# eminwux/kukeon

Hardware: AMD Instinct MI355X
Metric: agent_turns_per_sec (higher is better)
Workload: dtype bf16; 1 GPU; model=llama-3-8b, global_batch=64, seq_len=3584, parallelism=dp1, sessions_per_gpu_group=64, prompt_len=512, followup_len=256, decode_len=128

## Files before the change

kukeon_amd/ops/__init__.py:

```python
from __future__ import annotations

import torch

from . import reference

_C = None
_IMPORT_ERROR: Exception | None = None


def _load() -> None:
    global _C, _IMPORT_ERROR
    try:
        from kukeon_amd import _C as ext
    except Exception as e:
        _IMPORT_ERROR = e
    else:
        _C, _IMPORT_ERROR = ext, None


_load()


def native_available() -> bool:
    if _C is None:
        _load()
    return _C is not None


def _native():
    if _C is None:
        _load()
    if _C is None:
        raise RuntimeError(
            "kukeon_amd._C (gfx950 HIP extension) is not built but an op was "
            "called on a CUDA device. Run `python -m kukeon_amd.ops.build` "
            f"(import error: {_IMPORT_ERROR})")
    return _C


def _impl(t: torch.Tensor):
    return _native() if t.is_cuda else reference


def rmsnorm(out, input, weight, eps: float) -> None:
    _impl(input).rmsnorm(out, input, weight, eps)


def fused_add_rmsnorm(input, residual, weight, eps: float) -> None:
    _impl(input).fused_add_rmsnorm(input, residual, weight, eps)


def silu_mul(out, gate_up) -> None:
    _impl(gate_up).silu_mul(out, gate_up)


def rope_kv_append(qkv, k_cache, v_cache, cos_sin, positions, slot_mapping,
                   num_q_heads: int, num_kv_heads: int, head_dim: int,
                   block_table=None) -> None:
    if block_table is None:
        block_table = torch.empty(0, dtype=torch.int32, device=qkv.device)
    _impl(qkv).rope_kv_append(qkv, k_cache, v_cache, cos_sin, positions,
                              slot_mapping, num_q_heads, num_kv_heads,
                              head_dim, block_table)


def kv_copy_blocks(k_cache, v_cache, src, dst) -> None:
    _impl(k_cache).kv_copy_blocks(k_cache, v_cache, src, dst)


def decode_advance(ids, pos, seq_lens, tokens, ring, counter) -> None:
    _impl(ids).decode_advance(ids, pos, seq_lens, tokens, ring, counter)


def paged_attention(out, q, k_cache, v_cache, block_table, seq_lens,
                    q_offset: int, num_splits: int, scale: float,
                    tmp_out, tmp_ml) -> None:
    _impl(q).paged_attention(out, q, k_cache, v_cache, block_table, seq_lens,
                             q_offset, num_splits, scale, tmp_out, tmp_ml)


DECODE_ATTN_FUSED = __import__("os").environ.get(
    "KUKEON_DECODE_ATTN_FUSED", "1") != "0"


def paged_attention_rope(out, qkv, k_cache, v_cache, cos_sin, positions,
                         block_table, seq_lens, num_q_heads: int,
                         num_kv_heads: int, num_splits: int, scale: float,
                         tmp_out, tmp_ml) -> None:
    _impl(qkv).paged_attention_rope(out, qkv, k_cache, v_cache, cos_sin,
                                    positions, block_table, seq_lens,
                                    num_q_heads, num_kv_heads, num_splits,
                                    scale, tmp_out, tmp_ml)


def check_prefix_tiles(tiles, group: int) -> None:
    reference.check_prefix_tiles(tiles, group)


def paged_attention_shared(out, q, k_cache, v_cache, block_table, seq_lens,
                           q_offset: int, num_splits: int, scale: float,
                           tmp_out, tmp_ml, prefix_blocks, tiles,
                           prefix_splits: int) -> None:
    _impl(q).paged_attention_shared(out, q, k_cache, v_cache, block_table,
                                    seq_lens, q_offset, num_splits, scale,
                                    tmp_out, tmp_ml, prefix_blocks, tiles,
                                    prefix_splits)


def paged_attention_rope_shared(out, qkv, k_cache, v_cache, cos_sin,
                                positions, block_table, seq_lens,
                                num_q_heads: int, num_kv_heads: int,
                                num_splits: int, scale: float, tmp_out,
                                tmp_ml, prefix_blocks, tiles,
                                prefix_splits: int) -> None:
    _impl(qkv).paged_attention_rope_shared(
        out, qkv, k_cache, v_cache, cos_sin, positions, block_table,
        seq_lens, num_q_heads, num_kv_heads, num_splits, scale, tmp_out,
        tmp_ml, prefix_blocks, tiles, prefix_splits)


def prefill_attention(out, q, k_cache, v_cache, block_table, seq_lens,
                      q_starts, qb_seq, qb_start, q_offset: int,
                      scale: float) -> None:
    _impl(q).prefill_attention(out, q, k_cache, v_cache, block_table,
                               seq_lens, q_starts, qb_seq, qb_start, q_offset,
                               scale)


def sample(tokens, logits, temps, top_k, top_p, seed, workspace) -> None:
    _impl(logits).sample(tokens, logits, temps, top_k, top_p, seed, workspace)


_SKINNY_WS = {}
_SKINNY_WS_RETIRED = []
_USE_SKINNY = __import__("os").environ.get("KUKEON_SKINNY_GEMM", "0")
_FUSE_SILU = __import__("os").environ.get("KUKEON_FUSE_SILU", "0") == "1"


def _skinny_wins(rows: int, N: int, K: int) -> bool:
    if _USE_SKINNY == "off":
        return False
    return N == K == 4096


def _skinny5_wins(rows: int, N: int, K: int) -> bool:
    if _USE_SKINNY == "off":
        return False
    return (N, K) in ((4096, 14336), (8192, 28672))


def _skinny_kind(x: torch.Tensor, w: torch.Tensor, fused: bool):
    rows = x.shape[0]
    if not (x.is_cuda and x.dim() == 2 and rows <= 64
            and x.dtype == torch.bfloat16):
        return None
    N, K = w.shape
    if fused:
        from kukeon_amd import parallel
        if not (parallel.tp_size() == 1 and N % 2048 == 0 and N <= 8192):
            return None
    if (N % 128 == 0 and K % 128 == 0
            and (_USE_SKINNY == "5" or _skinny5_wins(rows, N, K))):
        return "v5"
    if (N % 64 == 0 and K % 32 == 0
            and (_USE_SKINNY == "1" or _skinny_wins(rows, N, K))):
        return "v1"
    return None


_SKINNY_SPLITK = {}


def _skinny_workspace(device: torch.device, kind: str, N: int,
                      K: int) -> torch.Tensor:
    splitk = _SKINNY_SPLITK.get((kind, N, K))
    if splitk is None:
        splitk = _SKINNY_SPLITK[kind, N, K] = _native().skinny_splitk(
            kind, N, K)
    need = 64 * N * splitk
    key = (device.index or 0)
    ws = _SKINNY_WS.get(key)
    if ws is None or ws.numel() < need:
        if ws is not None:
            _SKINNY_WS_RETIRED.append(ws)
        ws = torch.empty(need, dtype=torch.float32, device=device)
        _SKINNY_WS[key] = ws
    return ws


class Fp8Weight:

    __slots__ = ("q", "scale")

    def __init__(self, q: torch.Tensor, scale: torch.Tensor):
        assert q.dtype == torch.uint8 and q.dim() == 2
        assert scale.dtype == torch.float32 and scale.shape == (q.shape[0],)
        self.q = q
        self.scale = scale

    @property
    def shape(self):
        return tuple(self.q.shape)

    @property
    def device(self) -> torch.device:
        return self.q.device

    @property
    def is_cuda(self) -> bool:
        return self.q.is_cuda

    @property
    def nbytes(self) -> int:
        return self.q.numel() + 4 * self.scale.numel()


_W8_SCRATCH = {}
_W8_SCRATCH_RETIRED = []


def _w8_scratch(device: torch.device, numel: int) -> torch.Tensor:
    key = (device.index or 0)
    buf = _W8_SCRATCH.get(key)
    if buf is None or buf.numel() < numel:
        if buf is not None:
            _W8_SCRATCH_RETIRED.append(buf)
        buf = torch.empty(numel, dtype=torch.bfloat16, device=device)
        _W8_SCRATCH[key] = buf
    return buf


def quantize_weight(w: torch.Tensor) -> Fp8Weight:
    w = w.detach().contiguous()
    N, K = w.shape
    q = torch.empty(N, K, dtype=torch.uint8, device=w.device)
    scale = torch.empty(N, dtype=torch.float32, device=w.device)
    _impl(w).quantize_fp8_rows(q, scale, w)
    if w.is_cuda:
        _w8_scratch(w.device, N * K)
    return Fp8Weight(q, scale)


def dequantize_weight(fw: Fp8Weight, out: torch.Tensor = None) -> torch.Tensor:
    if out is None:
        out = torch.empty(fw.shape, dtype=torch.bfloat16, device=fw.device)
    _impl(fw.q).dequant_fp8_rows(out, fw.q, fw.scale)
    return out


def _w8_skinny(x: torch.Tensor, fw: Fp8Weight) -> bool:
    N, K = fw.shape
    return (x.is_cuda and x.dim() == 2 and 1 <= x.shape[0] <= 64
            and x.dtype == torch.bfloat16 and x.is_contiguous()
            and N % 64 == 0 and K % 64 == 0)


def _linear_w8(x: torch.Tensor, fw: Fp8Weight) -> torch.Tensor:
    if not x.is_cuda:
        return reference.linear_w8(x, fw.q, fw.scale)
    N, K = fw.shape
    if _w8_skinny(x, fw):
        out = torch.empty(x.shape[0], N, dtype=x.dtype, device=x.device)
        ws = _skinny_workspace(x.device, "w8", N, K)
        _native().skinny_gemm_w8(out, x, fw.q, fw.scale, ws)
        return out
    w = _w8_scratch(x.device, N * K)[:N * K].view(N, K)
    _native().dequant_fp8_rows(w, fw.q, fw.scale)
    return torch.nn.functional.linear(x, w)


def linear(x: torch.Tensor, w) -> torch.Tensor:
    if isinstance(w, Fp8Weight):
        return _linear_w8(x, w)
    kind = _skinny_kind(x, w, fused=False)
    if kind is None:
        return torch.nn.functional.linear(x, w)
    N, K = w.shape
    out = torch.empty(x.shape[0], N, dtype=x.dtype, device=x.device)
    ws = _skinny_workspace(x.device, kind, N, K)
    if kind == "v5":
        _native().skinny_gemm5(out, x, w, ws)
    else:
        _native().skinny_gemm(out, x, w, ws)
    return out


def linear_add_rmsnorm(x: torch.Tensor, w: torch.Tensor,
                       residual: torch.Tensor, norm_weight: torch.Tensor,
                       eps: float) -> torch.Tensor:
    if isinstance(w, Fp8Weight):
        from kukeon_amd import parallel
        N, K = w.shape
        if (_w8_skinny(x, w) and parallel.tp_size() == 1
                and N % 2048 == 0 and N <= 8192):
            normed = torch.empty(x.shape[0], N, dtype=x.dtype,
                                 device=x.device)
            ws = _skinny_workspace(x.device, "w8", N, K)
            _native().skinny_gemm_w8_fused_norm(normed, x, w.q, w.scale, ws,
                                                residual, norm_weight, eps)
            return normed
        kind = None
    else:
        kind = _skinny_kind(x, w, fused=True)
    if kind is None:
        from kukeon_amd import parallel
        h = parallel.tp_all_reduce(linear(x, w))
        fused_add_rmsnorm(h, residual, norm_weight, eps)
        return h
    N, K = w.shape
    normed = torch.empty(x.shape[0], N, dtype=x.dtype, device=x.device)
    if kind == "v5":
        ws = _skinny_workspace(x.device, "v5_fused", N, K)
        _native().skinny_gemm5_fused_norm(normed, x, w, ws, residual,
                                          norm_weight, eps)
    else:
        ws = _skinny_workspace(x.device, "v1", N, K)
        _native().skinny_gemm_fused_norm(normed, x, w, ws, residual,
                                         norm_weight, eps)
    return normed


def mlp_down_fused(gu: torch.Tensor, w: torch.Tensor,
                   residual: torch.Tensor, norm_weight: torch.Tensor,
                   eps: float) -> torch.Tensor:
    rows = gu.shape[0]
    N, K = w.shape
    if (_FUSE_SILU and not isinstance(w, Fp8Weight) and gu.dim() == 2
            and gu.shape[1] == 2 * K
            and _skinny_kind(gu, w, fused=True) == "v5"):
        ws = _skinny_workspace(gu.device, "v5_fused", N, K)
        normed = torch.empty(rows, N, dtype=gu.dtype, device=gu.device)
        _native().skinny_gemm5_silu_fused_norm(normed, gu, w, ws,
                                               residual, norm_weight, eps)
        return normed
    act = torch.empty(rows, K, dtype=gu.dtype, device=gu.device)
    silu_mul(act, gu)
    return linear_add_rmsnorm(act, w, residual, norm_weight, eps)


def moe_router_weights(wdense, logits, k: int) -> None:
    _impl(logits).moe_router_weights(wdense, logits, k)


def moe_dense_combine(out, y, wdense) -> None:
    _impl(y).moe_dense_combine(out, y, wdense)


def moe_gather_tokens(out, input, row_map) -> None:
    _impl(input).moe_gather_tokens(out, input, row_map)


def moe_scatter_tokens(out, input, inv_map, weights, top_k: int) -> None:
    _impl(input).moe_scatter_tokens(out, input, inv_map, weights, top_k)


def moe_route_sort(topk_w, row_map, inv_map, offsets, logits, k: int) -> None:
    _impl(logits).moe_route_sort(topk_w, row_map, inv_map, offsets, logits,
                                 k)


def moe_grouped_gemm(out, a, a_rows, w, offsets) -> None:
    if a_rows is None:
        a_rows = torch.empty(0, dtype=torch.int32, device=a.device)
    _impl(a).moe_grouped_gemm(out, a, a_rows, w, offsets)
```

kukeon_amd/ops/csrc/bindings.cpp:

```cpp
#include <torch/extension.h>

namespace kukeon {
void rmsnorm(torch::Tensor out, torch::Tensor input, torch::Tensor weight,
             double eps);
void fused_add_rmsnorm(torch::Tensor input, torch::Tensor residual,
                       torch::Tensor weight, double eps);
void silu_mul(torch::Tensor out, torch::Tensor gate_up);
void rope_kv_append(torch::Tensor qkv, torch::Tensor k_cache,
                    torch::Tensor v_cache, torch::Tensor cos_sin,
                    torch::Tensor positions, torch::Tensor slot_mapping,
                    int64_t num_q_heads, int64_t num_kv_heads,
                    int64_t head_dim, torch::Tensor block_table);
void decode_advance(torch::Tensor ids, torch::Tensor pos,
                    torch::Tensor seq_lens, torch::Tensor tokens,
                    torch::Tensor ring, torch::Tensor counter);
void kv_copy_blocks(torch::Tensor k_cache, torch::Tensor v_cache,
                    torch::Tensor src, torch::Tensor dst);
void paged_attention(torch::Tensor out, torch::Tensor q, torch::Tensor k_cache,
                     torch::Tensor v_cache, torch::Tensor block_table,
                     torch::Tensor seq_lens, int64_t q_offset,
                     int64_t num_splits, double scale, torch::Tensor tmp_out,
                     torch::Tensor tmp_ml);
void paged_attention_rope(torch::Tensor out, torch::Tensor qkv,
                          torch::Tensor k_cache, torch::Tensor v_cache,
                          torch::Tensor cos_sin, torch::Tensor positions,
                          torch::Tensor block_table, torch::Tensor seq_lens,
                          int64_t num_q_heads, int64_t num_kv_heads,
                          int64_t num_splits, double scale,
                          torch::Tensor tmp_out, torch::Tensor tmp_ml);
void paged_attention_shared(torch::Tensor out, torch::Tensor q,
                            torch::Tensor k_cache, torch::Tensor v_cache,
                            torch::Tensor block_table, torch::Tensor seq_lens,
                            int64_t q_offset, int64_t num_splits, double scale,
                            torch::Tensor tmp_out, torch::Tensor tmp_ml,
                            torch::Tensor prefix_blocks, torch::Tensor tiles,
                            int64_t prefix_splits);
void paged_attention_rope_shared(
    torch::Tensor out, torch::Tensor qkv, torch::Tensor k_cache,
    torch::Tensor v_cache, torch::Tensor cos_sin, torch::Tensor positions,
    torch::Tensor block_table, torch::Tensor seq_lens, int64_t num_q_heads,
    int64_t num_kv_heads, int64_t num_splits, double scale,
    torch::Tensor tmp_out, torch::Tensor tmp_ml, torch::Tensor prefix_blocks,
    torch::Tensor tiles, int64_t prefix_splits);
void prefill_attention(torch::Tensor out, torch::Tensor q,
                       torch::Tensor k_cache, torch::Tensor v_cache,
                       torch::Tensor block_table, torch::Tensor seq_lens,
                       torch::Tensor q_starts, torch::Tensor qb_seq,
                       torch::Tensor qb_start, int64_t q_offset, double scale);
void mfma_probe(torch::Tensor out, torch::Tensor a, torch::Tensor b);
void mfma_probe16(torch::Tensor out, torch::Tensor a, torch::Tensor b);
void mfma_probe16k(torch::Tensor out, torch::Tensor a, torch::Tensor b);
void skinny_gemm2(torch::Tensor out, torch::Tensor x, torch::Tensor w,
                  torch::Tensor ws);
void skinny_gemm5(torch::Tensor out, torch::Tensor x, torch::Tensor w,
                  torch::Tensor ws);
void skinny_gemm6(torch::Tensor out, torch::Tensor x, torch::Tensor w,
                  torch::Tensor ws);
void skinny_gemm5_silu_fused_norm(torch::Tensor normed, torch::Tensor gu,
                                  torch::Tensor w, torch::Tensor ws,
                                  torch::Tensor residual, torch::Tensor nw,
                                  double eps);
void skinny_gemm(torch::Tensor out, torch::Tensor x, torch::Tensor w,
                 torch::Tensor ws);
void glds_probe(torch::Tensor out, torch::Tensor src);
int64_t skinny_splitk(const std::string& kind, int64_t N, int64_t K);
void skinny_gemm5_fused_norm(torch::Tensor normed, torch::Tensor x,
                             torch::Tensor w, torch::Tensor ws,
                             torch::Tensor residual, torch::Tensor nw,
                             double eps);
void skinny_gemm_fused_norm(torch::Tensor normed, torch::Tensor x,
                            torch::Tensor w, torch::Tensor ws,
                            torch::Tensor residual, torch::Tensor nw,
                            double eps);
void skinny_gemm_w8(torch::Tensor out, torch::Tensor x, torch::Tensor q,
                    torch::Tensor scale, torch::Tensor ws);
void skinny_gemm_w8_fused_norm(torch::Tensor normed, torch::Tensor x,
                               torch::Tensor q, torch::Tensor scale,
                               torch::Tensor ws, torch::Tensor residual,
                               torch::Tensor nw, double eps);
void quantize_fp8_rows(torch::Tensor q, torch::Tensor scale, torch::Tensor w);
void dequant_fp8_rows(torch::Tensor out, torch::Tensor q,
                      torch::Tensor scale);
void sample(torch::Tensor tokens, torch::Tensor logits, torch::Tensor temps,
            torch::Tensor top_k, torch::Tensor top_p, torch::Tensor seed,
            torch::Tensor workspace);
void moe_router_weights(torch::Tensor wdense, torch::Tensor logits,
                        long K);
void moe_dense_combine(torch::Tensor out, torch::Tensor y,
                       torch::Tensor wdense);
void moe_gather_tokens(torch::Tensor out, torch::Tensor input,
                       torch::Tensor row_map);
void moe_scatter_tokens(torch::Tensor out, torch::Tensor input,
                        torch::Tensor row_map, torch::Tensor weights,
                        int64_t top_k);
void moe_route_sort(torch::Tensor topk_w, torch::Tensor row_map,
                    torch::Tensor inv_map, torch::Tensor offsets,
                    torch::Tensor logits, long K);
void moe_grouped_gemm(torch::Tensor out, torch::Tensor a,
                      torch::Tensor a_rows, torch::Tensor w,
                      torch::Tensor offsets);
}

PYBIND11_MODULE(TORCH_EXTENSION_NAME, m) {
  m.def("rmsnorm", &kukeon::rmsnorm, "RMSNorm (bf16, gfx950)");
  m.def("fused_add_rmsnorm", &kukeon::fused_add_rmsnorm,
        "residual += input; input = rmsnorm(residual)");
  m.def("silu_mul", &kukeon::silu_mul, "out = silu(gate)*up from fused [T,2I]");
  m.def("rope_kv_append", &kukeon::rope_kv_append,
        "in-place NEOX RoPE on fused qkv + paged KV append");
  m.def("kv_copy_blocks", &kukeon::kv_copy_blocks,
        "cache[l, dst[i]] = cache[l, src[i]] for K and V, all layers, one "
        "launch");
  m.def("paged_attention", &kukeon::paged_attention,
        "decode paged attention (GQA, split-KV)");
  m.def("paged_attention_rope", &kukeon::paged_attention_rope,
        "decode paged attention with RoPE + KV append folded in");
  m.def("paged_attention_shared", &kukeon::paged_attention_shared,
        "decode paged attention, shared prefix blocks read once per tile of "
        "rows");
  m.def("paged_attention_rope_shared", &kukeon::paged_attention_rope_shared,
        "paged_attention_rope, shared prefix blocks read once per tile of "
        "rows");
  m.def("prefill_attention", &kukeon::prefill_attention,
        "varlen causal paged prefill attention (MFMA)");
  m.def("mfma_probe", &kukeon::mfma_probe,
        "32x32x16 bf16 MFMA fragment-layout probe");
  m.def("mfma_probe16", &kukeon::mfma_probe16,
        "16x16x32 bf16 MFMA fragment-layout probe");
  m.def("mfma_probe16k", &kukeon::mfma_probe16k,
        "16x16x16 (K=16) bf16 MFMA fragment-layout probe");
  m.def("skinny_gemm6", &kukeon::skinny_gemm6,
        "decode GEMM v6 (barrier-free register-x pipeline)");
  m.def("skinny_gemm5_silu_fused_norm",
        &kukeon::skinny_gemm5_silu_fused_norm,
        "silu(gate)*up + down GEMM + reduce + add + RMSNorm fused");
  m.def("skinny_gemm5", &kukeon::skinny_gemm5,
        "full-line W stream via wave-private LDS image (v5)");
  m.def("skinny_gemm2", &kukeon::skinny_gemm2,
        "G-walk hand-counted weight-streaming GEMM (v2)");
  m.def("skinny_gemm", &kukeon::skinny_gemm,
        "weight-streaming decode GEMM (M<=64)");
  m.def("skinny_splitk", &kukeon::skinny_splitk,
        "split-K factor the skinny launcher of `kind` (v1, v2, v5, v5_fused, "
        "v6, w8) uses for [N, K]; host-only",
        py::arg("kind"), py::arg("N"), py::arg("K"));
  m.def("glds_probe", &kukeon::glds_probe,
        "asm global_lds round-trip validator");
  m.def("skinny_gemm5_fused_norm", &kukeon::skinny_gemm5_fused_norm,
        "skinny5 + fused split-K reduce + residual add + RMSNorm");
  m.def("skinny_gemm_fused_norm", &kukeon::skinny_gemm_fused_norm,
        "skinny GEMM + split-K reduce + residual add + RMSNorm");
  m.def("skinny_gemm_w8", &kukeon::skinny_gemm_w8,
        "W8A16 decode GEMM: (x @ fp8(q)^T) * scale, M<=64");
  m.def("skinny_gemm_w8_fused_norm", &kukeon::skinny_gemm_w8_fused_norm,
        "W8A16 decode GEMM + split-K reduce + residual add + RMSNorm");
  m.def("quantize_fp8_rows", &kukeon::quantize_fp8_rows,
        "bf16 [N,K] -> e4m3fn bytes + per-row f32 scale (amax/448)");
  m.def("dequant_fp8_rows", &kukeon::dequant_fp8_rows,
        "out = bf16(fp8(q) * scale[n])");
  m.def("sample", &kukeon::sample, "top-k/top-p/temperature sampling");
  m.def("decode_advance", &kukeon::decode_advance,
        "on-device decode cursor advance (self-advancing graph)");
  m.def("moe_gather_tokens", &kukeon::moe_gather_tokens, "MoE permute");
  m.def("moe_router_weights", &kukeon::moe_router_weights,
        "softmax top-K renorm -> dense [T,E] weights, one launch");
  m.def("moe_dense_combine", &kukeon::moe_dense_combine,
        "out = sum_e w[t,e]*y[e,t,:], zero-weight experts skipped");
  m.def("moe_scatter_tokens", &kukeon::moe_scatter_tokens,
        "MoE unpermute + weighted combine");
  m.def("moe_route_sort", &kukeon::moe_route_sort,
        "top-k routing + stable expert sort on the device, one launch");
  m.def("moe_grouped_gemm", &kukeon::moe_grouped_gemm,
        "out[r] = a[a_rows[r]] @ w[e].T, expert row ranges from device");
}
```

kukeon_amd/ops/csrc/prefill_attn.hip:

```cpp
#include "attn_frag.h"
#include <torch/extension.h>
#include <c10/hip/HIPStream.h>

namespace kukeon {

template <int BS, bool FP8>
__global__ __launch_bounds__(256, 1) void prefill_attn_kernel(
    unsigned short* __restrict__ out,
    const unsigned short* __restrict__ q,
    const void* __restrict__ k_cache,
    const void* __restrict__ v_cache,
    const int* __restrict__ block_table,
    const int* __restrict__ seq_lens,
    const int* __restrict__ q_starts,
    const int* __restrict__ qb_seq,
    const int* __restrict__ qb_start,
    long q_stride, long q_offset, int Hq, int Hk, int max_blocks,
    int out_stride, float scale) {
  constexpr int D = 128;
  constexpr int KVT = 32;
  __shared__ __align__(16) unsigned short kbuf[KVT * D];
  __shared__ __align__(16) unsigned short vtbuf[D * KVT];

  const int s = qb_seq[blockIdx.x];
  const int qb0 = qb_start[blockIdx.x];
  const int hk = blockIdx.y;
  const int ctx = seq_lens[s];
  const int abs_start = q_starts[2 * s];
  const int row0 = q_starts[2 * s + 1] + qb0;
  const int qlen = ctx - abs_start;
  const int qn = min(32, qlen - qb0);
  if (qn <= 0) return;
  const int G = Hq / Hk;
  const int wid = threadIdx.x / WAVE;
  const int lane = threadIdx.x & (WAVE - 1);
  const int hi = lane >> 5;
  const int qcol = lane & 31;
  const int h_local = blockIdx.z * 4 + wid;
  const bool active = h_local < G;
  const int head = hk * G + (active ? h_local : 0);

  const int q_abs = abs_start + qb0 + min(qcol, qn - 1);

  unsigned int qfrag[8][4];
  {
    const long qrow = row0 + min(qcol, qn - 1);
    const unsigned short* qp = q + qrow * q_stride + q_offset + (long)head * D;
#pragma unroll
    for (int st = 0; st < 8; ++st) {
      const uint4 v = *reinterpret_cast<const uint4*>(qp + st * 16 + hi * 8);
      qfrag[st][0] = v.x; qfrag[st][1] = v.y;
      qfrag[st][2] = v.z; qfrag[st][3] = v.w;
    }
  }

  float m = -INFINITY, l_acc = 0.f;
  f32x16_t oacc[4] = {{}, {}, {}, {}};

  const int kv_limit = min(ctx, abs_start + qb0 + qn);
  const int ntiles = (kv_limit + KVT - 1) / KVT;
  const int nblocks = (ctx + BS - 1) / BS;

  for (int ti = 0; ti < ntiles; ++ti) {
    const int kvbase = ti * KVT;
    {
      __syncthreads();
      const auto* kc = reinterpret_cast<const kv_elem_t<FP8>*>(k_cache);
      const auto* vc = reinterpret_cast<const kv_elem_t<FP8>*>(v_cache);
      const int tok = threadIdx.x >> 3;
      const int d0 = (threadIdx.x & 7) * 16;
      const int kvpos = kvbase + tok;
      const int bidx = min(kvpos / BS, nblocks - 1);
      const int pblk = block_table[(long)s * max_blocks + bidx];
      const long koff = (((long)pblk * Hk + hk) * BS + (kvpos % BS)) * D;
      const int swz = (tok & 15) << 4;
#pragma unroll
      for (int c = 0; c < 2; ++c) {
        const int byte = tok * 256 + (((d0 + c * 8) * 2) ^ swz);
        *reinterpret_cast<uint4*>(reinterpret_cast<char*>(kbuf) + byte) =
            load_kv8(kc + koff + d0 + c * 8);
      }
      const int kp = threadIdx.x >> 4;
      const int vd0 = (threadIdx.x & 15) * 8;
      const int vpos0 = kvbase + 2 * kp;
      const int vpos1 = vpos0 + 1;
      const int vb0 = min(vpos0 / BS, nblocks - 1);
      const int vb1 = min(vpos1 / BS, nblocks - 1);
      const long voff0 =
          (((long)block_table[(long)s * max_blocks + vb0] * Hk + hk) * BS +
           (vpos0 % BS)) * D;
      const long voff1 =
          (((long)block_table[(long)s * max_blocks + vb1] * Hk + hk) * BS +
           (vpos1 % BS)) * D;
      uint4 r0 = load_kv8(vc + voff0 + vd0);
      uint4 r1 = load_kv8(vc + voff1 + vd0);
      if (vpos0 >= ctx) r0 = uint4{0, 0, 0, 0};
      if (vpos1 >= ctx) r1 = uint4{0, 0, 0, 0};
      const unsigned int* a0 = reinterpret_cast<const unsigned int*>(&r0);
      const unsigned int* a1 = reinterpret_cast<const unsigned int*>(&r1);
#pragma unroll
      for (int j = 0; j < 8; ++j) {
        const unsigned short e0 = (a0[j >> 1] >> ((j & 1) * 16)) & 0xffffu;
        const unsigned short e1 = (a1[j >> 1] >> ((j & 1) * 16)) & 0xffffu;
        const unsigned int packed = (unsigned)e0 | ((unsigned)e1 << 16);
        const int d = vd0 + j;
        const int byte = d * 64 + ((4 * kp) ^ ((d & 3) << 4));
        *reinterpret_cast<unsigned int*>(
            reinterpret_cast<char*>(vtbuf) + byte) = packed;
      }
      __syncthreads();
    }
    if (!active) continue;

    f32x16_t sacc = {};
#pragma unroll
    for (int st = 0; st < 8; ++st) {
      const int row = qcol;
      const int byte = row * 256 + (((st * 16 + hi * 8) * 2) ^ ((row & 15) << 4));
      const uint4 kf = *reinterpret_cast<const uint4*>(
          reinterpret_cast<const char*>(kbuf) + byte);
      sacc = __builtin_amdgcn_mfma_f32_32x32x16_bf16(
          as_frag(kf.x, kf.y, kf.z, kf.w),
          as_frag(qfrag[st][0], qfrag[st][1], qfrag[st][2], qfrag[st][3]),
          sacc, 0, 0, 0);
    }

    float sv[16];
    float tmax = -INFINITY;
#pragma unroll
    for (int r = 0; r < 16; ++r) {
      const int kvrow = (r & 3) + 8 * (r >> 2) + 4 * hi;
      const int kvpos = kvbase + kvrow;
      const bool valid = (kvpos <= q_abs) && (kvpos < ctx);
      sv[r] = valid ? sacc[r] * scale : -INFINITY;
      tmax = fmaxf(tmax, sv[r]);
    }
    tmax = fmaxf(tmax, __shfl_xor(tmax, 32, WAVE));
    const float mn = fmaxf(m, tmax);
    const float alpha = (m == -INFINITY) ? 0.f : __expf(m - mn);
    m = mn;
    float psum = 0.f;
    float p[16];
#pragma unroll
    for (int r = 0; r < 16; ++r) {
      p[r] = (sv[r] == -INFINITY) ? 0.f : __expf(sv[r] - mn);
      psum += p[r];
    }
    psum += __shfl_xor(psum, 32, WAVE);
    l_acc = l_acc * alpha + psum;
#pragma unroll
    for (int db = 0; db < 4; ++db)
#pragma unroll
      for (int r = 0; r < 16; ++r) oacc[db][r] *= alpha;

    unsigned int cp[8];
#pragma unroll
    for (int j = 0; j < 8; ++j) cp[j] = cvtpk_bf16(p[2 * j], p[2 * j + 1]);
    unsigned int pb[2][4];
#pragma unroll
    for (int c = 0; c < 2; ++c) {
      const int b0 = 4 * c;
      auto s1 = __builtin_amdgcn_permlane32_swap(cp[b0 + 0], cp[b0 + 2],
                                                 false, false);
      auto s2 = __builtin_amdgcn_permlane32_swap(cp[b0 + 1], cp[b0 + 3],
                                                 false, false);
      pb[c][0] = s1[0]; pb[c][1] = s2[0];
      pb[c][2] = s1[1]; pb[c][3] = s2[1];
    }

#pragma unroll
    for (int db = 0; db < 4; ++db) {
      const int d = db * 32 + qcol;
#pragma unroll
      for (int c = 0; c < 2; ++c) {
        const int byte = d * 64 + (((c * 32) + hi * 16) ^ ((d & 3) << 4));
        const uint4 vf = *reinterpret_cast<const uint4*>(
            reinterpret_cast<const char*>(vtbuf) + byte);
        oacc[db] = __builtin_amdgcn_mfma_f32_32x32x16_bf16(
            as_frag(vf.x, vf.y, vf.z, vf.w),
            as_frag(pb[c][0], pb[c][1], pb[c][2], pb[c][3]),
            oacc[db], 0, 0, 0);
      }
    }
  }

  if (!active || qcol >= qn) return;
  const float inv = l_acc > 0.f ? 1.f / l_acc : 0.f;
  unsigned short* orow = out + (long)(row0 + qcol) * out_stride +
                         (long)head * D;
#pragma unroll
  for (int db = 0; db < 4; ++db) {
#pragma unroll
    for (int quad = 0; quad < 4; ++quad) {
      const int d = db * 32 + quad * 8 + 4 * hi;
      const unsigned int w0 = cvtpk_bf16(oacc[db][quad * 4 + 0] * inv,
                                          oacc[db][quad * 4 + 1] * inv);
      const unsigned int w1 = cvtpk_bf16(oacc[db][quad * 4 + 2] * inv,
                                          oacc[db][quad * 4 + 3] * inv);
      *reinterpret_cast<uint2*>(orow + d) = uint2{w0, w1};
    }
  }
}

void prefill_attention(torch::Tensor out, torch::Tensor q,
                       torch::Tensor k_cache, torch::Tensor v_cache,
                       torch::Tensor block_table, torch::Tensor seq_lens,
                       torch::Tensor q_starts, torch::Tensor qb_seq,
                       torch::Tensor qb_start, int64_t q_offset, double scale) {
  const int Hk = k_cache.size(1);
  const int BS = k_cache.size(2);
  const int D = k_cache.size(3);
  const int Hq = out.size(1) / D;
  const int G = Hq / Hk;
  const int nqb = qb_seq.size(0);
  if (nqb == 0) return;
  TORCH_CHECK(D == 128, "only head_dim=128 supported");
  TORCH_CHECK(BS == 16, "kv block size must be 16");
  TORCH_CHECK(q_starts.dim() == 2 && q_starts.size(1) == 2);
  TORCH_CHECK(qb_seq.scalar_type() == torch::kInt32);
  auto stream = c10::hip::getCurrentHIPStream().stream();
  dim3 grid(nqb, Hk, (G + 3) / 4);
  const bool fp8 = k_cache.scalar_type() == torch::kUInt8;
#define PF_LAUNCH(FP8_)                                                      \
  prefill_attn_kernel<16, FP8_><<<grid, 256, 0, stream>>>(                   \
      reinterpret_cast<unsigned short*>(out.data_ptr()),                     \
      reinterpret_cast<const unsigned short*>(q.data_ptr()),                 \
      k_cache.data_ptr(), v_cache.data_ptr(), block_table.data_ptr<int>(),   \
      seq_lens.data_ptr<int>(), q_starts.data_ptr<int>(),                    \
      qb_seq.data_ptr<int>(), qb_start.data_ptr<int>(), q.stride(0),         \
      q_offset, Hq, Hk, (int)block_table.size(1), (int)out.stride(0),        \
      (float)scale)
  if (fp8) { PF_LAUNCH(true); } else { PF_LAUNCH(false); }
#undef PF_LAUNCH
  HIP_CHECK_KERNEL();
}

}
```

Before: 51.24 turns/s.

## Double-buffer KV tiles in prefill attention and remap blocks across XCDs

Adds a pipelined variant of the prefill attention kernel. It keeps two LDS buffers for the K and transposed-V tiles and prefetches the next tiles' block-table entries and raw KV into registers while the current tile's QK MFMAs run. It also raises launch_bounds occupancy to 2 blocks per CU and optionally remaps block IDs so that consecutive logical tiles land on the same XCD for better L2 locality. Both paths are on by default behind env flags. The cost is doubled shared memory and more live registers, and prefill is only one part of an agent-turn workload.

```diff
diff --git a/kukeon_amd/ops/__init__.py b/kukeon_amd/ops/__init__.py
--- a/kukeon_amd/ops/__init__.py
+++ b/kukeon_amd/ops/__init__.py
@@ -119,12 +119,25 @@
         tmp_ml, prefix_blocks, tiles, prefix_splits)
 
 
+PREFILL_ATTN_PIPELINED = __import__("os").environ.get(
+    "KUKEON_PREFILL_ATTN_PIPELINED", "1") != "0"
+PREFILL_ATTN_XCD_REMAP = __import__("os").environ.get(
+    "KUKEON_PREFILL_ATTN_XCD", "1") != "0"
+
+
 def prefill_attention(out, q, k_cache, v_cache, block_table, seq_lens,
                       q_starts, qb_seq, qb_start, q_offset: int,
                       scale: float) -> None:
-    _impl(q).prefill_attention(out, q, k_cache, v_cache, block_table,
-                               seq_lens, q_starts, qb_seq, qb_start, q_offset,
-                               scale)
+    if not q.is_cuda:
+        reference.prefill_attention(out, q, k_cache, v_cache, block_table,
+                                    seq_lens, q_starts, qb_seq, qb_start,
+                                    q_offset, scale)
+        return
+    _native().prefill_attention(out, q, k_cache, v_cache, block_table,
+                                seq_lens, q_starts, qb_seq, qb_start,
+                                q_offset, scale, PREFILL_ATTN_PIPELINED,
+                                PREFILL_ATTN_PIPELINED
+                                and PREFILL_ATTN_XCD_REMAP)
 
 
 def sample(tokens, logits, temps, top_k, top_p, seed, workspace) -> None:
diff --git a/kukeon_amd/ops/csrc/bindings.cpp b/kukeon_amd/ops/csrc/bindings.cpp
--- a/kukeon_amd/ops/csrc/bindings.cpp
+++ b/kukeon_amd/ops/csrc/bindings.cpp
@@ -46,7 +46,8 @@
                        torch::Tensor k_cache, torch::Tensor v_cache,
                        torch::Tensor block_table, torch::Tensor seq_lens,
                        torch::Tensor q_starts, torch::Tensor qb_seq,
-                       torch::Tensor qb_start, int64_t q_offset, double scale);
+                       torch::Tensor qb_start, int64_t q_offset, double scale,
+                       bool pipelined, bool xcd_remap);
 void mfma_probe(torch::Tensor out, torch::Tensor a, torch::Tensor b);
 void mfma_probe16(torch::Tensor out, torch::Tensor a, torch::Tensor b);
 void mfma_probe16k(torch::Tensor out, torch::Tensor a, torch::Tensor b);
diff --git a/kukeon_amd/ops/csrc/prefill_attn.hip b/kukeon_amd/ops/csrc/prefill_attn.hip
--- a/kukeon_amd/ops/csrc/prefill_attn.hip
+++ b/kukeon_amd/ops/csrc/prefill_attn.hip
@@ -4,8 +4,19 @@
 
 namespace kukeon {
 
-template <int BS, bool FP8>
-__global__ __launch_bounds__(256, 1) void prefill_attn_kernel(
+template <bool FP8>
+using kv_raw8_t = std::conditional_t<FP8, uint2, uint4>;
+DEV_INLINE uint4 load_raw8(const unsigned short* p) {
+  return *reinterpret_cast<const uint4*>(p);
+}
+DEV_INLINE uint2 load_raw8(const unsigned char* p) {
+  return *reinterpret_cast<const uint2*>(p);
+}
+DEV_INLINE uint4 raw8_to_bf16x8(uint4 r) { return r; }
+DEV_INLINE uint4 raw8_to_bf16x8(uint2 r) { return fp8x8_to_bf16x8(r); }
+
+template <int BS, bool FP8, bool PIPE>
+__global__ __launch_bounds__(256, PIPE ? 2 : 1) void prefill_attn_kernel(
     unsigned short* __restrict__ out,
     const unsigned short* __restrict__ q,
     const void* __restrict__ k_cache,
@@ -16,15 +27,26 @@
     const int* __restrict__ qb_seq,
     const int* __restrict__ qb_start,
     long q_stride, long q_offset, int Hq, int Hk, int max_blocks,
-    int out_stride, float scale) {
+    int out_stride, float scale, int xcd_remap) {
   constexpr int D = 128;
   constexpr int KVT = 32;
-  __shared__ __align__(16) unsigned short kbuf[KVT * D];
-  __shared__ __align__(16) unsigned short vtbuf[D * KVT];
-
-  const int s = qb_seq[blockIdx.x];
-  const int qb0 = qb_start[blockIdx.x];
-  const int hk = blockIdx.y;
+  constexpr int NBUF = PIPE ? 2 : 1;
+  __shared__ __align__(16) unsigned short kbufs[NBUF][KVT * D];
+  __shared__ __align__(16) unsigned short vtbufs[NBUF][D * KVT];
+
+  int qb = blockIdx.x, hk = blockIdx.y, zg = blockIdx.z;
+  if (xcd_remap) {
+    const int nqb = gridDim.x, nhk = gridDim.y;
+    const int total = nqb * nhk * (int)gridDim.z;
+    const int id = qb + nqb * (hk + nhk * zg);
+    const int xcd = id & 7;
+    const int logical = xcd * (total >> 3) + min(xcd, total & 7) + (id >> 3);
+    qb = logical % nqb;
+    hk = (logical / nqb) % nhk;
+    zg = logical / (nqb * nhk);
+  }
+  const int s = qb_seq[qb];
+  const int qb0 = qb_start[qb];
   const int ctx = seq_lens[s];
   const int abs_start = q_starts[2 * s];
   const int row0 = q_starts[2 * s + 1] + qb0;
@@ -36,7 +58,7 @@
   const int lane = threadIdx.x & (WAVE - 1);
   const int hi = lane >> 5;
   const int qcol = lane & 31;
-  const int h_local = blockIdx.z * 4 + wid;
+  const int h_local = zg * 4 + wid;
   const bool active = h_local < G;
   const int head = hk * G + (active ? h_local : 0);
 
@@ -61,9 +83,68 @@
   const int ntiles = (kv_limit + KVT - 1) / KVT;
   const int nblocks = (ctx + BS - 1) / BS;
 
+  const int st_tok = threadIdx.x >> 3;
+  const int st_d0 = (threadIdx.x & 7) * 16;
+  const int st_kp = threadIdx.x >> 4;
+  const int st_vd0 = (threadIdx.x & 15) * 8;
+  kv_raw8_t<FP8> kraw[2], vraw[2];
+  int blk = 0;
+  static_assert(KVT == 2 * BS, "tile = two cache blocks");
+  const int st_b = threadIdx.x >> 7;
+  auto resolve = [&](int t) {
+    blk = block_table[(long)s * max_blocks + min(2 * t + st_b, nblocks - 1)];
+  };
+  auto issue = [&](int t) {
+    const auto* kc = reinterpret_cast<const kv_elem_t<FP8>*>(k_cache);
+    const auto* vc = reinterpret_cast<const kv_elem_t<FP8>*>(v_cache);
+    const long base = ((long)blk * Hk + hk) * BS;
+    const auto* kp = kc + (base + (st_tok % BS)) * D + st_d0;
+    kraw[0] = load_raw8(kp);
+    kraw[1] = load_raw8(kp + 8);
+    const auto* vp = vc + (base + ((2 * st_kp) % BS)) * D + st_vd0;
+    vraw[0] = load_raw8(vp);
+    vraw[1] = load_raw8(vp + D);
+  };
+  auto write_images = [&](int t, unsigned short* kbuf, unsigned short* vtbuf) {
+    const int swz = (st_tok & 15) << 4;
+#pragma unroll
+    for (int c = 0; c < 2; ++c) {
+      const int byte = st_tok * 256 + (((st_d0 + c * 8) * 2) ^ swz);
+      *reinterpret_cast<uint4*>(reinterpret_cast<char*>(kbuf) + byte) =
+          raw8_to_bf16x8(kraw[c]);
+    }
+    uint4 r0 = raw8_to_bf16x8(vraw[0]);
+    uint4 r1 = raw8_to_bf16x8(vraw[1]);
+    const int vpos0 = t * KVT + 2 * st_kp;
+    if (vpos0 >= ctx) r0 = uint4{0, 0, 0, 0};
+    if (vpos0 + 1 >= ctx) r1 = uint4{0, 0, 0, 0};
+    const unsigned int* a0 = reinterpret_cast<const unsigned int*>(&r0);
+    const unsigned int* a1 = reinterpret_cast<const unsigned int*>(&r1);
+#pragma unroll
+    for (int j = 0; j < 8; ++j) {
+      const unsigned short e0 = (a0[j >> 1] >> ((j & 1) * 16)) & 0xffffu;
+      const unsigned short e1 = (a1[j >> 1] >> ((j & 1) * 16)) & 0xffffu;
+      const unsigned int packed = (unsigned)e0 | ((unsigned)e1 << 16);
+      const int d = st_vd0 + j;
+      const int byte = d * 64 + ((4 * st_kp) ^ ((d & 3) << 4));
+      *reinterpret_cast<unsigned int*>(
+          reinterpret_cast<char*>(vtbuf) + byte) = packed;
+    }
+  };
+  if constexpr (PIPE) {
+    resolve(0);
+    issue(0);
+    if (ntiles > 1) resolve(1);
+    write_images(0, kbufs[0], vtbufs[0]);
+    if (ntiles > 1) issue(1);
+    if (ntiles > 2) resolve(2);
+  }
+
   for (int ti = 0; ti < ntiles; ++ti) {
     const int kvbase = ti * KVT;
-    {
+    unsigned short* const kbuf = kbufs[PIPE ? (ti & 1) : 0];
+    unsigned short* const vtbuf = vtbufs[PIPE ? (ti & 1) : 0];
+    if constexpr (!PIPE) {
       __syncthreads();
       const auto* kc = reinterpret_cast<const kv_elem_t<FP8>*>(k_cache);
       const auto* vc = reinterpret_cast<const kv_elem_t<FP8>*>(v_cache);
@@ -109,20 +190,36 @@
             reinterpret_cast<char*>(vtbuf) + byte) = packed;
       }
       __syncthreads();
-    }
-    if (!active) continue;
+      if (!active) continue;
+    } else {
+      __syncthreads();
+    }
 
     f32x16_t sacc = {};
-#pragma unroll
-    for (int st = 0; st < 8; ++st) {
-      const int row = qcol;
-      const int byte = row * 256 + (((st * 16 + hi * 8) * 2) ^ ((row & 15) << 4));
-      const uint4 kf = *reinterpret_cast<const uint4*>(
-          reinterpret_cast<const char*>(kbuf) + byte);
-      sacc = __builtin_amdgcn_mfma_f32_32x32x16_bf16(
-          as_frag(kf.x, kf.y, kf.z, kf.w),
-          as_frag(qfrag[st][0], qfrag[st][1], qfrag[st][2], qfrag[st][3]),
-          sacc, 0, 0, 0);
+    if (!PIPE || active) {
+#pragma unroll
+      for (int st = 0; st < 8; ++st) {
+        const int row = qcol;
+        const int byte =
+            row * 256 + (((st * 16 + hi * 8) * 2) ^ ((row & 15) << 4));
+        const uint4 kf = *reinterpret_cast<const uint4*>(
+            reinterpret_cast<const char*>(kbuf) + byte);
+        sacc = __builtin_amdgcn_mfma_f32_32x32x16_bf16(
+            as_frag(kf.x, kf.y, kf.z, kf.w),
+            as_frag(qfrag[st][0], qfrag[st][1], qfrag[st][2], qfrag[st][3]),
+            sacc, 0, 0, 0);
+      }
+    }
+
+    if constexpr (PIPE) {
+      if (ti + 1 < ntiles) {
+        write_images(ti + 1, kbufs[(ti + 1) & 1], vtbufs[(ti + 1) & 1]);
+        if (ti + 2 < ntiles) {
+          issue(ti + 2);
+          if (ti + 3 < ntiles) resolve(ti + 3);
+        }
+      }
+      if (!active) continue;
     }
 
     float sv[16];
@@ -206,7 +303,8 @@
                        torch::Tensor k_cache, torch::Tensor v_cache,
                        torch::Tensor block_table, torch::Tensor seq_lens,
                        torch::Tensor q_starts, torch::Tensor qb_seq,
-                       torch::Tensor qb_start, int64_t q_offset, double scale) {
+                       torch::Tensor qb_start, int64_t q_offset, double scale,
+                       bool pipelined, bool xcd_remap) {
   const int Hk = k_cache.size(1);
   const int BS = k_cache.size(2);
   const int D = k_cache.size(3);
@@ -221,16 +319,20 @@
   auto stream = c10::hip::getCurrentHIPStream().stream();
   dim3 grid(nqb, Hk, (G + 3) / 4);
   const bool fp8 = k_cache.scalar_type() == torch::kUInt8;
-#define PF_LAUNCH(FP8_)                                                      \
-  prefill_attn_kernel<16, FP8_><<<grid, 256, 0, stream>>>(                   \
+#define PF_LAUNCH(FP8_, PIPE_)                                               \
+  prefill_attn_kernel<16, FP8_, PIPE_><<<grid, 256, 0, stream>>>(            \
       reinterpret_cast<unsigned short*>(out.data_ptr()),                     \
       reinterpret_cast<const unsigned short*>(q.data_ptr()),                 \
       k_cache.data_ptr(), v_cache.data_ptr(), block_table.data_ptr<int>(),   \
       seq_lens.data_ptr<int>(), q_starts.data_ptr<int>(),                    \
       qb_seq.data_ptr<int>(), qb_start.data_ptr<int>(), q.stride(0),         \
       q_offset, Hq, Hk, (int)block_table.size(1), (int)out.stride(0),        \
-      (float)scale)
-  if (fp8) { PF_LAUNCH(true); } else { PF_LAUNCH(false); }
+      (float)scale, (int)xcd_remap)
+  if (pipelined) {
+    if (fp8) { PF_LAUNCH(true, true); } else { PF_LAUNCH(false, true); }
+  } else {
+    if (fp8) { PF_LAUNCH(true, false); } else { PF_LAUNCH(false, false); }
+  }
 #undef PF_LAUNCH
   HIP_CHECK_KERNEL();
 }
```

Measured after the change: 51.59 turns/s (median of 6 runs). No clear change (+0.7%).
